# vliu15/3d-brain-tumor-segmentation

Measured on AMD Instinct MI355X. Metric: training volumes/sec (2ch x 128^3), higher is better.
Workload: dtype f32; 1 GPU; BASELINE configs[1]: 2ch x 128^3, batch 1 per GPU, fp32, full fwd+bwd with Dice+KL+L2 VAE loss + Dice metric + TF-form Adam; CLI-default model (base_filters=32, depth=4, groups=8, reduction=8; 42,174,773 params); parallelism=dp1, global_batch=1

## Files before the change

3d-brain-tumor-segmentation_amd/csrc/groupnorm.hip:

```cpp
#include <stdlib.h>
#include "common.h"
#include "bts_internal.h"
#include "finalize_parts.h"

#define GN_BLOCKS_MAX 256

struct GnGeom {
  int N, C, G, cg, mode;
  long V;
  long E;
  long L;
  int B;
  long span;
  int generic;
};

static int gn_geom(GnGeom& g, int N, long V, int C, int G, int mode) {
  if (N <= 0 || V <= 0 || C <= 0 || G <= 0) return BTS_ERR_SHAPE;
  if (C < G || C % G != 0) return BTS_ERR_SHAPE;
  g.N = N; g.C = C; g.G = G; g.cg = C / G; g.mode = mode; g.V = V; g.E = V * C; g.L = g.E / G;
  if (g.E % G != 0) return BTS_ERR_UNSUPPORTED;
  g.generic = (C % 4 != 0 || (C & (C - 1)) != 0 || C > 1024 || g.L % 4 != 0) ? 1 : 0;
  const long unit = (mode == BTS_GN_SLAB) ? g.L : g.E;
  const int units = (mode == BTS_GN_SLAB) ? N * G : N;
// ... 550 lines not shown
                                                           int C, int G, int cg, int lddy, int mode, int relu) {
  const long f0 = blockIdx.x * (long)blockDim.x + threadIdx.x;
  const int cph = (int)((f0 * 4) % C);
  const bool fixed = ((long)gridDim.x * 1024) % C == 0;
  for (long f = f0; f < total4; f += (long)gridDim.x * blockDim.x) {
    const long i = f * 4;
    const long n = i / E;
    const long r = i - n * E;
    const int c = fixed ? cph : (int)(r % C);
    const long pix = i / C;
    const f32x4 v = *reinterpret_cast<const f32x4*>(x + i);
    const f32x4 d = *reinterpret_cast<const f32x4*>(dy + pix * lddy + c);
    const int gsl = (int)(r / L);
    f32x4 o;
#pragma unroll
    for (int e = 0; e < 4; ++e) {
      const int g = (mode == BTS_GN_SLAB) ? gsl : (c + e) / cg;
      const int idx = (mode == BTS_GN_SLAB) ? g * cg + ((c + e) % cg) : (c + e);
      const float rs = rstd[n * G + g];
      const float xh = (v[e] - mean[n * G + g]) * rs;
      float de = d[e];
      const float ga = gamma[idx];
      if (relu && !(xh * ga + beta[idx] > 0.f)) de = 0.f;
      o[e] = (de * ga - c1[n * G + g] - xh * c2[n * G + g]) * rs;
    }
    *reinterpret_cast<f32x4*>(dx + i) = o;
  }
}

bool bts_gn_slab_blocks_(int N, long V, int C, int G, int* B, long* span) {
  GnGeom g;
  if (gn_geom(g, N, V, C, G, BTS_GN_SLAB) != BTS_OK || g.generic) return false;
  *B = g.B;
  *span = g.span;
  return true;
}
__global__ __launch_bounds__(256) void gn_bwd_apply_slab_stream_kernel(const float* __restrict__ x, const float* __restrict__ dy,
                                                                       float* __restrict__ dx, const float* __restrict__ gamma,
                                                                       const float* __restrict__ beta, const float* __restrict__ mean,
                                                                       const float* __restrict__ rstd, const float* __restrict__ c1,
                                                                       const float* __restrict__ c2, long chunks_per_unit, int cpb,
                                                                       int C, int cg, int G, int relu, int lddy) {
  const long chunk0 = (long)blockIdx.x * cpb;
  const long unit = chunk0 / chunks_per_unit;
  const int g = (int)(unit % G);
  const float m = mean[unit], rs = rstd[unit], k1 = c1[unit], k2 = c2[unit];
  const int c = (threadIdx.x * 4) % C;
  float ga[4], be[4];
#pragma unroll
  for (int e = 0; e < 4; ++e) {
    const int idx = g * cg + ((c + e) % cg);
    ga[e] = gamma[idx];
    be[e] = beta[idx];
  }
  const long off = chunk0 * 1024 + threadIdx.x * 4;
  const long vpc = 1024 / C;
  const long doff = (chunk0 * vpc + (threadIdx.x * 4) / C) * lddy + c;
  const long dstep = vpc * lddy;
  auto one = [&](const f32x4 v, const f32x4 d) {
    f32x4 o;
#pragma unroll
    for (int e = 0; e < 4; ++e) {
      const float xh = (v[e] - m) * rs;
      float de = d[e];
      if (relu && !(xh * ga[e] + be[e] > 0.f)) de = 0.f;
      o[e] = (de * ga[e] - k1 - xh * k2) * rs;
    }
    return o;
  };
  int k = 0;
  for (; k + 1 < cpb; k += 2) {
    const f32x4 v0 = *reinterpret_cast<const f32x4*>(x + off + (long)k * 1024);
    const f32x4 d0 = *reinterpret_cast<const f32x4*>(dy + doff + (long)k * dstep);
    const f32x4 v1 = *reinterpret_cast<const f32x4*>(x + off + (long)(k + 1) * 1024);
    const f32x4 d1 = *reinterpret_cast<const f32x4*>(dy + doff + (long)(k + 1) * dstep);
    *reinterpret_cast<f32x4*>(dx + off + (long)k * 1024) = one(v0, d0);
    *reinterpret_cast<f32x4*>(dx + off + (long)(k + 1) * 1024) = one(v1, d1);
  }
  for (; k < cpb; ++k) {
    const f32x4 v0 = *reinterpret_cast<const f32x4*>(x + off + (long)k * 1024);
    const f32x4 d0 = *reinterpret_cast<const f32x4*>(dy + doff + (long)k * dstep);
    *reinterpret_cast<f32x4*>(dx + off + (long)k * 1024) = one(v0, d0);
  }
}

extern "C" int bts_gn_bwd(const float* x, const float* dy, float* dx, const float* gamma, const float* beta,
                          const float* mean, const float* rstd, float* dgamma, float* dbeta, void* workspace,
                          long workspace_bytes, int N, long V, int C, int lddy, int G, int mode, int relu,
                          int accumulate_params, hipStream_t stream) {
  GnGeom g;
  int r = gn_geom(g, N, V, C, G, mode);
  if (r != BTS_OK) return r;
  if (lddy < C) return BTS_ERR_ALIGN;
  if (workspace == nullptr) return BTS_ERR_WORKSPACE;
  if (g.generic || lddy % 4 != 0) {
    if (workspace_bytes < (long)N * G * 2 * 4 + 64) return BTS_ERR_WORKSPACE;
    float* gc1 = reinterpret_cast<float*>(workspace);
    float* gc2 = gc1 + (long)N * G;
    (void)hipGetLastError(); hipLaunchKernelGGL(gn_bwd_group_generic_kernel, dim3(N * G), dim3(256), 0, stream, x, dy, gamma, beta, mean, rstd, gc1, gc2,
                       g.E, g.L, C, G, g.cg, lddy, mode, relu);
    BTS_LAUNCH_CHECK();
    (void)hipGetLastError(); hipLaunchKernelGGL(gn_bwd_param_generic_kernel, dim3(C), dim3(256), 0, stream, x, dy, gamma, beta, mean, rstd, dgamma, dbeta,
                       N, g.E, g.L, C, G, g.cg, lddy, mode, relu, accumulate_params);
    BTS_LAUNCH_CHECK();
    const long total = (long)N * g.E;
    int gb = (int)((total + 255) / 256);
    if (gb > 8192) gb = 8192;
    (void)hipGetLastError(); hipLaunchKernelGGL(gn_bwd_apply_generic_kernel, dim3(gb), dim3(256), 0, stream, x, dy, dx, gamma, beta, mean, rstd, gc1, gc2,
                       total, g.E, g.L, C, G, g.cg, lddy, mode, relu);
    BTS_LAUNCH_CHECK();
    return BTS_OK;
  }
  if ((((uintptr_t)x) & 15) || (((uintptr_t)dy) & 15) || (((uintptr_t)dx) & 15)) return BTS_ERR_ALIGN;
  const long part_bytes = bts_gn_workspace(N, V, C, G, mode);
  const long extra = (long)N * C * 2 * 8 + (long)N * G * 2 * 4 + 64;
  if (workspace_bytes < part_bytes + extra) return BTS_ERR_WORKSPACE;
  double* partial = reinterpret_cast<double*>(workspace);
  double* scratch = reinterpret_cast<double*>(reinterpret_cast<char*>(workspace) + ((part_bytes + 15) & ~15L));
  float* c1 = reinterpret_cast<float*>(scratch + (long)N * C * 2);
  float* c2 = c1 + (long)N * G;
  const bool slab = (mode == BTS_GN_SLAB);
  (void)hipGetLastError(); hipLaunchKernelGGL(gn_bwd_reduce_kernel, dim3(g.B, slab ? N * G : N), dim3(256), 0, stream, x, dy, gamma, beta, mean,
                     rstd, partial, g.E, g.L, g.span, C, G, g.cg, lddy, mode, relu);
  BTS_LAUNCH_CHECK();
  if (slab && g.cg <= 256 && 256 % g.cg == 0) {
    (void)hipGetLastError(); hipLaunchKernelGGL(gn_bwd_finalize_slab_kernel, dim3(G), dim3(256), 0, stream, partial, gamma, dgamma, dbeta, c1, c2, N, G, g.B,
                       g.cg, (double)g.L, accumulate_params);
    BTS_LAUNCH_CHECK();
  } else {
    (void)hipGetLastError(); hipLaunchKernelGGL(gn_bwd_finalize_a_kernel, dim3((N * C + 3) / 4), dim3(256), 0, stream, partial, scratch, N, g.B, C, G, mode);
    BTS_LAUNCH_CHECK();
    (void)hipGetLastError(); hipLaunchKernelGGL(gn_bwd_finalize_kernel, dim3(1), dim3(256), 0, stream, gamma, dgamma, dbeta, c1, c2, scratch, N, C, G,
                       (double)g.L, accumulate_params);
    BTS_LAUNCH_CHECK();
  }
  if (slab && g.L % 1024 == 0 && 1024 % C == 0) {
    const long cpu = g.L / 1024;
    const int cpb = gn_stream_cpb(cpu);
    const long nblk = (long)N * G * cpu / cpb;
    if (nblk <= 0x7fffffffL) {
      (void)hipGetLastError(); hipLaunchKernelGGL(gn_bwd_apply_slab_stream_kernel, dim3((unsigned)nblk), dim3(256), 0, stream, x, dy, dx, gamma, beta,
                         mean, rstd, c1, c2, cpu, cpb, C, g.cg, G, relu, lddy);
      BTS_LAUNCH_CHECK();
      return BTS_OK;
    }
  }
  const long total4 = (long)N * g.E / 4;
  int blocks = (int)((total4 + 255) / 256);
  if (blocks > 8192) blocks = 8192;
  (void)hipGetLastError(); hipLaunchKernelGGL(gn_bwd_apply_kernel, dim3(blocks), dim3(256), 0, stream, x, dy, dx, gamma, beta, mean, rstd, c1, c2,
                     total4, g.E, g.L, C, G, g.cg, lddy, mode, relu);
  BTS_LAUNCH_CHECK();
  return BTS_OK;
}

extern "C" long bts_gn_bwd_workspace(int N, long V, int C, int G, int mode) {
  const long p = bts_gn_workspace(N, V, C, G, mode);
  if (p < 0) return -1;
  return ((p + 15) & ~15L) + (long)N * C * 2 * 8 + (long)N * G * 2 * 4 + 64;
}
```

3d-brain-tumor-segmentation_amd/layers/resnet.py:

```python
import os

import torch

from .. import ops
from ._base import Layer, Tensor, as_tensor, check_data_format, current_tape, gn_mode_of
from .group_norm import GroupNormalization


class ResnetBlock(Layer):
    def __init__(self, filters, data_format='channels_last', groups=8, reduction=2, l2_scale=1e-5, name=None):
        super(ResnetBlock, self).__init__(name=name)
        self.data_format = check_data_format(data_format)
        self.config = {'filters': filters, 'data_format': data_format, 'reduction': reduction, 'l2_scale': l2_scale,
                       'groups': groups}
        if filters % reduction != 0:
            raise ValueError('Reduction ratio, {}, must be a factor of number of channels, {}.'.format(reduction, filters))
        self.filters = filters
        self.groups = groups
        self.reduction = reduction
        self.l2_scale = l2_scale
        self.norm1 = self.track(GroupNormalization(groups=groups, axis=-1, beta_initializer='zeros',
                                                   gamma_initializer='ones', beta_regularizer=l2_scale,
                                                   gamma_regularizer=l2_scale, name=self.name + '/gn1',
                                                   semantics=gn_mode_of(data_format)))
# ... 70 lines not shown
            return res_, gap_, hbuf_, ch_

        if gate is not None:
            gate.wait_stream(main)
            with torch.cuda.stream(gate):
                res, gap, hbuf, ch = gate_branch(None)
            x.t.record_stream(gate)
            for t in (res, gap, hbuf, ch):
                t.record_stream(main)
        if fused is None:
            if slab:
                c1, m1, r1 = ops.conv_fwd_gn(K3, x.t, wp_c1, self.conv1_b.t, f, g, self.norm1.epsilon)
            else:
                c1 = ops.conv_fwd(K3, x.t, wp_c1, self.conv1_b.t, f)
        if gate is None:
            res, gap, hbuf, ch = gate_branch(res)
        if m1 is None:
            m1, r1 = ops.gn_stats(c1, g, self.norm1._mode, self.norm1.epsilon)
        a = ops.gn_apply(c1, self.norm1.gamma.t, self.norm1.beta.t, m1, r1, g, self.norm1._mode, True)
        if slab:
            c2, m2, r2 = ops.conv_fwd_gn(K3, a, wp_c2, self.conv2_b.t, f, g, self.norm2.epsilon)
        else:
            c2 = ops.conv_fwd(K3, a, wp_c2, self.conv2_b.t, f)
            m2, r2 = ops.gn_stats(c2, g, self.norm2._mode, self.norm2.epsilon)
        if gate is not None:
            main.wait_stream(gate)
        if out is None:
            out = Tensor(torch.empty((n, d, h, w, f), dtype=torch.float32, device=x.t.device))
        wsp = self.spatial_k.t.reshape(-1)
        sp = ops.block_epilogue_fwd(res, c2, out.t, wsp, ch, self.norm2.gamma.t, self.norm2.beta.t, m2, r2, g, self.norm2._mode)
        out.cf = self.data_format == 'channels_first'
        tape = current_tape()
        if tape is not None:
            def backward():
                self._backward(x, out, res, gap, hbuf, ch, sp, c1, m1, r1, a, c2, m2, r2, dup_start, dup_shift)
            tape.record(backward)
        return out

    def _backward(self, x, out, res, gap, hbuf, ch, sp, c1, m1, r1, a, c2, m2, r2, dup_start, dup_shift):
        dout = out.grad
        if dout is None:
            return
        f, g = self.filters, self.groups
        cin = x.shape[-1]
        K1, K3 = ops.K1, ops.K3S1
        n1, n2 = self.norm1, self.norm2
        from .group_norm import group_norm_backward
        gw1, a1 = self.se_w1.grad_slot()
        gw2, a2 = self.se_w2.grad_slot()
        gws, a3 = self.spatial_k.grad_slot()
        main = torch.cuda.current_stream()
        gate = ops.side_stream('gate')
        fused = None
        if n2._mode == ops.GN_SLAB and n2.gamma is not None and n2.beta is not None and os.environ.get('BTS_FUSE_BLOCK_BWD', '1') != '0':
            fused = self._fused_gate_gn2_backward(dout, res, c2, sp, gap, hbuf, ch, m2, r2, (gw1, a1), (gw2, a2), (gws, a3))

        def gate_backward():
            acc_ = a1
            if not (a1 == a2 == a3):
                for buf, ac in ((gw1, a1), (gw2, a2), (gws, a3)):
                    if not ac:
                        ops.fill(buf, 0.0)
                acc_ = True
            return ops.se_bwd(dout, res, sp, gap, hbuf, ch, self.se_w1.t, self.se_w2.t, self.spatial_k.t.reshape(-1), gw1, gw2,
                              gws.reshape(-1), accumulate_params=acc_)

        if fused is not None:
            dres, dc2 = fused
            gate = None
        elif gate is not None:
            gate.wait_stream(main)
            with torch.cuda.stream(gate):
                dres = gate_backward()
            for t in (dout, res, sp, gap, hbuf, ch):
                t.record_stream(gate)
            dres.record_stream(main)
        if fused is None:
            dc2 = group_norm_backward(n2, c2, dout, n2.gamma.t, n2.beta.t, m2, r2, True)
        wpb2 = self.packed('c2_b', K3, ops.ROLE_BWD, self.conv2_k, f, f)
        da = torch.empty_like(a)
        ops.conv_bwd_data(K3, dc2, wpb2, da, False)
        _wgrad(K3, a, dc2, self.conv2_k, self.conv2_b)
        del dc2
        dc1 = group_norm_backward(n1, c1, da, n1.gamma.t, n1.beta.t, m1, r1, True)
        del da
        need_dx = x.requires_grad
        if fused is not None:
            pass
        elif gate is None:
            dres = gate_backward()
        else:
            main.wait_stream(gate)
        if need_dx:
            dx, acc = x.grad_slot()
            wpb1 = self.packed('c1_b', K3, ops.ROLE_BWD, self.conv1_k, self.cin_ref, f, cin, dup_start, dup_shift)
            wpbp = self.packed('pt_b', K1, ops.ROLE_BWD, self.ptwise_k, self.cin_ref, f, cin, dup_start, dup_shift)
            ops.conv_bwd_data_pair(dc1, wpb1, dres, wpbp, dx, acc)
        _wgrad(K3, x.t, dc1, self.conv1_k, self.conv1_b, dup_start, dup_shift)
        del dc1
        _wgrad(K1, x.t, dres, self.ptwise_k, self.ptwise_b, dup_start, dup_shift)

    def _fused_gate_gn2_backward(self, dout, res, c2, sp, gap, hbuf, ch, m2, r2, s1, s2, s3):
        n2 = self.norm2
        (gw1, a1), (gw2, a2), (gws, a3) = s1, s2, s3
        if not (torch.is_tensor(dout) and dout.shape[-1] == self.filters):
            return None
        if not ops.block_bwd_takes(res, self.se_w1.t.shape[1], n2.groups, dout, c2):
            return None
        dg, ag = n2.gamma.grad_slot()
        db, ab = n2.beta.grad_slot()
        if not (a1 == a2 == a3):
            for buf, ac in ((gw1, a1), (gw2, a2), (gws, a3)):
                if not ac:
                    ops.fill(buf, 0.0)
            a1 = True
        if ag != ab:
            if not ag:
                ops.fill(dg, 0.0)
            if not ab:
                ops.fill(db, 0.0)
            ag = True
        out = ops.block_bwd(dout, res, c2, sp, gap, hbuf, ch, self.se_w1.t, self.se_w2.t, self.spatial_k.t.reshape(-1), n2.gamma.t, n2.beta.t,
                            m2, r2, n2.groups, gw1, gw2, gws.reshape(-1), dg, db, accumulate_gate_params=a1, accumulate_norm_params=ag)
        if out is None:
            raise RuntimeError('ops.block_bwd declined a block ops.block_bwd_takes accepted')
        return out

    def get_config(self):
        return self.config


def _wgrad(kind, x, dy, kparam, bparam, dup_start=0, dup_shift=0):
    side = ops.side_stream()
    if side is None:
        return _wgrad_here(kind, x, dy, kparam, bparam, dup_start, dup_shift)
    side.wait_stream(torch.cuda.current_stream())
    with torch.cuda.stream(side):
        _wgrad_here(kind, x, dy, kparam, bparam, dup_start, dup_shift)
    for t in (x, dy):
        t.record_stream(side)


def _wgrad_here(kind, x, dy, kparam, bparam, dup_start=0, dup_shift=0):
    dw, aw = kparam.grad_slot()
    db, ab = (None, aw) if bparam is None else bparam.grad_slot()
    if bparam is not None and aw != ab:
        if not aw:
            ops.fill(dw, 0.0)
        if not ab:
            ops.fill(db, 0.0)
        aw = True
    if kind == ops.K3S2T:
        ops.conv_bwd_weight(kind, x, dy, dw, None, accumulate=aw)
        if bparam is not None:
            ops.colsum(dy, sum_over_n=True, out=db, accumulate=aw)
    else:
        ops.conv_bwd_weight(kind, x, dy, dw, db, dup_start, dup_shift, accumulate=aw)
```

3d-brain-tumor-segmentation_amd/ops.py:

```python
import ctypes
import weakref

import numpy as np
import torch

from ._lib import ERRORS, lib

K1, K3S1, K3S2, K3S2T = 0, 1, 2, 3
ROLE_FWD, ROLE_BWD = 0, 1
FLAG_SIGMOID, FLAG_ACCUM = 1, 2
GN_SLAB, GN_CHANNEL = 0, 1

_workspaces = {}

_CFG = {0: '2,1,4,1', 1: '2,2,4,1', 2: '1,2,2,2', 3: '1,1,2,2', 4: '1,1,4,1'}


_VARIANTS = {33: {1: '<0,5>', 2: '<0,4>', 3: '<1,5>', 4: '<1,4>'},
             32: {1: '<3x3x3>', 2: '<1x1x1>'}}


def kernel_symbol(sym, detail=False):
    var, sym = sym >> 16, sym & 0xffff
    if var and detail and sym in _VARIANTS:
        return kernel_symbol(sym) + _VARIANTS[sym].get(var, '<%d>' % var)
    if sym == 20:
        return 'upm_kernel'
    if sym == 21:
        return 'k1s_kernel'
    if sym == 22:
        return 'dsc_kernel'
    if sym == 23:
        return 'wino_kernel'
    if sym == 24:
        return 'wgw_kernel'
    if sym == 25:
        return 'c2_kernel'
    if sym == 26:
        return 'k1w_kernel'
    if sym == 27:
        return 'w3_kernel'
    if sym == 30:
        return 'lp_conv_s1_kernel'
    if sym == 31:
        return 'lp_conv_gather_kernel'
    if sym == 32:
        return 'lp_wgrad_kernel'
    if sym == 33:
        return 'lp_s1d_kernel'
    if sym == 34:
        return 'lp_k1_kernel'
    if sym == 35:
        return 'lp_up_kernel'
    if sym == 36:
        return 'lp_wgs_kernel'
    if sym == 37:
        return 'lp_wgd_kernel'
    if sym == 38:
        return 'lp_s1z_kernel'
    if sym == 39:
        return 'lp_s2t_kernel'
    if sym == 40:
        return 'lp_c2_kernel'
    if sym >= 100:
        return 'wgrad_kernel<%d,%d>' % ((sym - 100) >> 2, (sym - 100) & 3)
    return 'igemm_kernel<%s,%d>' % (_CFG[sym & 7], 4 if sym & 8 else 1)


def profile_enable(on):
    lib().call('bts_profile_enable', 1 if on else 0)


def profile_records(detail=False):
    L = lib()
    out = []
    sym, fl, ms = ctypes.c_int(), ctypes.c_double(), ctypes.c_float()
    for i in range(L._bts_profile_count()):
        L.call('bts_profile_get', i, ctypes.byref(sym), ctypes.byref(fl), ctypes.byref(ms))
        out.append((kernel_symbol(sym.value, detail), fl.value, ms.value))
    return out


def conv_bwd_data_pair(dy, wp_bwd, dy2, wp2_bwd, dx, accumulate):
    n, d, h, w, cin = dx.shape
    cout = dy.shape[4]
    nb = lib().query('bts_conv3d_bwd_data_pair_workspace', n, d, h, w, cin, cout)
    ws = workspace(nb, dy.device) if nb > 0 else None
    lib().call('bts_conv3d_bwd_data_pair', _p(dy), _p(wp_bwd), _p(dy2), _p(wp2_bwd), _p(dx), _p(ws), nb, n, d, h, w, cin,
               ld_of(dx), cout, ld_of(dy), ld_of(dy2), FLAG_ACCUM if accumulate else 0, _stream())
    return dx


def conv_flops(kind, n, d, h, w, cin, cout):
    v = n * d * h * w
    if kind == K1:
        return 2.0 * cin * cout * v
    if kind == K3S2:
        return 2.0 * 27 * cin * cout * (v // 8)
    return 2.0 * 27 * cin * cout * v


def _p(t):
    return None if t is None else ctypes.c_void_p(t.data_ptr())


def _stream():
    return ctypes.c_void_p(torch.cuda.current_stream().cuda_stream)


_side = {}
_side_enabled = True


_fence = {}


def step_fence(kind='train', depth=2):
    import os
    if not torch.cuda.is_available() or os.environ.get('BTS_STEP_FENCE') == '0':
        return
    key = (torch.cuda.current_device(), kind)
    q = _fence.setdefault(key, [])
    while len(q) >= depth:
        q.pop(0).synchronize()
# ... 176 lines not shown
    return c1, res


def conv_fwd_gn(kind, x, wp, bias, cout, groups, eps):
    n, d, h, w, cin = x.shape
    y = torch.empty(conv_out_shape(kind, x.shape, cout), dtype=torch.float32, device=x.device)
    mean = torch.empty(n * groups, dtype=torch.float32, device=x.device)
    rstd = torch.empty(n * groups, dtype=torch.float32, device=x.device)
    nb = lib().query('bts_conv3d_fwd_gn_workspace', kind, n, d, h, w, cin, cout, groups)
    ws = workspace(nb, x.device)
    lib().call('bts_conv3d_fwd_gn', kind, _p(x), _p(wp), _p(bias), _p(y), _p(ws), nb, n, d, h, w, cin, ld_of(x), cout, groups,
               float(eps), _p(mean), _p(rstd), _stream())
    return y, mean, rstd


def conv_fwd_fused2_gn(x, wp3, bias3, wp1, bias1, cout, groups, eps):
    n, d, h, w, cin = x.shape
    if not lib()._bts_conv3d_fwd_can_fuse(n, d, h, w, cin, cout):
        return None
    c1 = torch.empty((n, d, h, w, cout), dtype=torch.float32, device=x.device)
    res = torch.empty_like(c1)
    mean = torch.empty(n * groups, dtype=torch.float32, device=x.device)
    rstd = torch.empty(n * groups, dtype=torch.float32, device=x.device)
    nb = lib().query('bts_conv3d_fwd_gn_workspace', K3S1, n, d, h, w, cin, cout, groups)
    ws = workspace(nb, x.device)
    lib().call('bts_conv3d_fwd_fused2_gn', _p(x), _p(wp3), _p(bias3), _p(c1), _p(wp1), _p(bias1), _p(res), _p(ws), nb, n, d, h, w,
               cin, ld_of(x), cout, cout, groups, float(eps), _p(mean), _p(rstd), _stream())
    return c1, res, mean, rstd


def conv_bwd_data(kind, dy, wp_bwd, dx, accumulate):
    n, d, h, w, cin = dx.shape
    cout = dy.shape[4]
    nb = lib().query('bts_conv3d_bwd_data_workspace', kind, n, d, h, w, cin, cout)
    ws = workspace(nb, dy.device) if nb > 0 else None
    if True:
        lib().call('bts_conv3d_bwd_data', kind, _p(dy), _p(wp_bwd), _p(dx), _p(ws), nb, n, d, h, w, cin, ld_of(dx), cout,
                   ld_of(dy), FLAG_ACCUM if accumulate else 0, _stream())
    return dx


def conv_bwd_weight(kind, x, dy, dw, db, dup_start=0, dup_shift=0, accumulate=False):
    n, d, h, w, cin = x.shape
    cout = dy.shape[4]
    nb = lib().query('bts_conv3d_bwd_weight_workspace', kind, n, d, h, w, cin, cout)
    ws = workspace(nb, x.device)
    if True:
        lib().call('bts_conv3d_bwd_weight', kind, _p(x), _p(dy), _p(dw), _p(db), _p(ws), nb, n, d, h, w, cin, ld_of(x),
                   cout, ld_of(dy), dup_start, dup_shift, 1 if accumulate else 0, _stream())


def gn_stats(x, groups, mode, eps=1e-5):
    if not x.is_contiguous():
        raise RuntimeError('GroupNormalization statistics need a dense tensor')
    n, c = x.shape[0], x.shape[4]
    v = x.shape[1] * x.shape[2] * x.shape[3]
    nb = lib().query('bts_gn_workspace', n, v, c, groups, mode)
    ws = workspace(nb, x.device)
    mean = torch.empty(n * groups, dtype=torch.float32, device=x.device)
    rstd = torch.empty_like(mean)
    lib().call('bts_gn_stats', _p(x), _p(mean), _p(rstd), _p(ws), nb, n, v, c, groups, mode, eps, _stream())
    return mean, rstd


def gn_apply(x, gamma, beta, mean, rstd, groups, mode, relu, out=None):
    n, c = x.shape[0], x.shape[4]
    v = x.shape[1] * x.shape[2] * x.shape[3]
    if out is None:
        out = torch.empty_like(x)
    lib().call('bts_gn_apply', _p(x), _p(out), _p(gamma), _p(beta), _p(mean), _p(rstd), n, v, c, ld_of(out), groups, mode,
               1 if relu else 0, _stream())
    return out


def gn_bwd(x, dy, gamma, beta, mean, rstd, dgamma, dbeta, groups, mode, relu, accumulate_params=False):
    n, c = x.shape[0], x.shape[4]
    v = x.shape[1] * x.shape[2] * x.shape[3]
    nb = lib().query('bts_gn_bwd_workspace', n, v, c, groups, mode)
    ws = workspace(nb, x.device)
    dx = torch.empty_like(x)
    lib().call('bts_gn_bwd', _p(x), _p(dy), _p(dx), _p(gamma), _p(beta), _p(mean), _p(rstd), _p(dgamma), _p(dbeta), _p(ws),
               nb, n, v, c, ld_of(dy), groups, mode, 1 if relu else 0, 1 if accumulate_params else 0, _stream())
    return dx


def colsum(x, scale=1.0, sum_over_n=False, out=None, accumulate=False):
    n, c = x.shape[0], x.shape[-1]
    rows = x.numel() // (n * c)
    ld = ld_of(x) if x.dim() == 5 else x.stride(-2)
    nb = lib().query('bts_colsum_workspace', n, rows, c)
    ws = workspace(nb, x.device)
    if out is None:
        out = torch.empty((c,) if sum_over_n else (n, c), dtype=torch.float32, device=x.device)
    lib().call('bts_colsum', _p(x), _p(out), _p(ws), nb, n, rows, c, ld, float(scale), 1 if sum_over_n else 0,
               1 if accumulate else 0, _stream())
    return out


def se_mlp_fwd(gap, w1, w2):
    n, f = gap.shape
    r = w1.shape[1]
    h = torch.empty((n, r), dtype=torch.float32, device=gap.device)
    ch = torch.empty((n, f), dtype=torch.float32, device=gap.device)
    lib().call('bts_se_mlp_fwd', _p(gap), _p(w1), _p(w2), _p(h), _p(ch), n, f, r, _stream())
    return h, ch


def block_epilogue_fwd(res, c2, out, wsp, ch, gamma, beta, mean, rstd, groups, mode):
    n, f = res.shape[0], res.shape[4]
    v = res.shape[1] * res.shape[2] * res.shape[3]
    sp = torch.empty(n * v, dtype=torch.float32, device=res.device)
    lib().call('bts_block_epilogue_fwd', _p(res), _p(c2), _p(out), _p(sp), _p(wsp), _p(ch), _p(gamma), _p(beta), _p(mean),
               _p(rstd), n, v, f, ld_of(out), groups, mode, _stream())
    return sp


def se_bwd(dout, res, sp, gap, h, ch, w1, w2, wsp, dw1, dw2, dwsp, accumulate_params=False):
    n, f = res.shape[0], res.shape[4]
    v = res.shape[1] * res.shape[2] * res.shape[3]
    r = w1.shape[1]
    nb = lib().query('bts_se_bwd_workspace', n, v, f, r)
    ws = workspace(nb, res.device)
    dres = torch.empty_like(res)
    ds = torch.empty(n * v, dtype=torch.float32, device=res.device)
    dgap = torch.empty((n, f), dtype=torch.float32, device=res.device)
    lib().call('bts_se_bwd', _p(dout), _p(res), _p(sp), _p(gap), _p(h), _p(ch), _p(w1), _p(w2), _p(wsp), _p(dres), _p(ds),
               _p(dgap), _p(dw1), _p(dw2), _p(dwsp), _p(ws), nb, n, v, f, r, ld_of(dout), 1 if accumulate_params else 0,
               _stream())
    return dres


def block_bwd_takes(res, r, groups, dout, c2):
    n, f = res.shape[0], res.shape[4]
    v = res.shape[1] * res.shape[2] * res.shape[3]
    return (lib().probe('bts_block_bwd_workspace', n, v, f, r, groups) >= 0 and ld_of(dout) % 4 == 0 and res.is_contiguous()
            and c2.is_contiguous() and all(t.data_ptr() % 16 == 0 for t in (dout, res, c2)))


def block_bwd(dout, res, c2, sp, gap, h, ch, w1, w2, wsp, gamma, beta, mean, rstd, groups, dw1, dw2, dwsp, dgamma, dbeta,
              accumulate_gate_params=False, accumulate_norm_params=False):
    n, f = res.shape[0], res.shape[4]
    v = res.shape[1] * res.shape[2] * res.shape[3]
    r = w1.shape[1]
    nb = lib().probe('bts_block_bwd_workspace', n, v, f, r, groups)
    if not block_bwd_takes(res, r, groups, dout, c2):
        return None
    ws = workspace(nb, res.device)
    dres = torch.empty_like(res)
    dc2 = torch.empty_like(c2)
    ds = torch.empty(n * v, dtype=torch.float32, device=res.device)
    dgap = torch.empty((n, f), dtype=torch.float32, device=res.device)
    lib().call('bts_block_bwd', _p(dout), ld_of(dout), _p(res), _p(c2), _p(sp), _p(gap), _p(h), _p(ch), _p(w1), _p(w2), _p(wsp), _p(gamma), _p(beta),
               _p(mean), _p(rstd), _p(dres), _p(dc2), _p(ds), _p(dgap), _p(dw1), _p(dw2), _p(dwsp), _p(dgamma), _p(dbeta), _p(ws), nb, n, v, f, r,
               groups, 1 if accumulate_gate_params else 0, 1 if accumulate_norm_params else 0, _stream())
    return dres, dc2


def dropout_mask(shape, rate, seed, device):
    m = torch.empty(shape, dtype=torch.uint8, device=device)
    lib().call('bts_dropout_mask', _p(m), m.numel(), float(rate), int(seed) & (2 ** 64 - 1), _stream())
    return m


def dropout_apply(x, mask, rate):
    y = torch.empty_like(x)
    lib().call('bts_dropout_apply', _p(x), _p(mask), _p(y), x.numel(), float(rate), _stream())
# ... 851 lines not shown
```

include/bts_hip.h:

```cpp
#ifndef BTS_HIP_H
#define BTS_HIP_H
#include <stdint.h>
#ifdef __cplusplus
extern "C" {
#endif

typedef struct ihipStream_t* bts_stream_t;

#define BTS_OK 0
#define BTS_ERR_SHAPE (-1)
#define BTS_ERR_ALIGN (-2)
#define BTS_ERR_UNSUPPORTED (-3)
#define BTS_ERR_WORKSPACE (-4)
#define BTS_ERR_RCCL_BASE (-100)

#define BTS_CONV_K1 0
#define BTS_CONV_K3S1 1
#define BTS_CONV_K3S2 2
#define BTS_CONV_K3S2T 3
#define BTS_ROLE_FWD 0
#define BTS_ROLE_BWD_DATA 1
#define BTS_CONV_FLAG_SIGMOID 1
#define BTS_CONV_FLAG_ACCUM 2

#define BTS_GN_SLAB 0
#define BTS_GN_CHANNEL 1


long bts_conv_packed_floats(int kind, int role, int Cin, int Cout);
int bts_conv_pack(int kind, int role, const float* w, float* wp, int Cin_ref, int Cout, int Cin_slab, int dup_start,
                  int dup_shift, bts_stream_t stream);
long bts_conv_pack_desc_bytes(void);
long bts_conv_pack_desc(void* host_table, int index, long first_block, int kind, int role, const float* w, float* wp,
                        int Cin_ref, int Cout, int Cin_slab, int dup_start, int dup_shift);
int bts_conv_pack_batch(const void* table_dev, const void* table_host, int n, long total_blocks, bts_stream_t stream);
long bts_conv_pack_generation(void);
int bts_conv_pack_forget(const float* wp);
long bts_conv3d_fwd_workspace(int kind, int N, int D, int H, int W, int Cin, int Cout);
int bts_conv3d_fwd(int kind, const float* x, const float* wp_fwd, const float* bias, float* y, void* workspace,
                   long workspace_bytes, int N, int D, int H, int W, int Cin, int ldx, int Cout, int ldy, int flags,
                   bts_stream_t stream);
int bts_conv3d_fwd_can_fuse(int N, int D, int H, int W, int Cin, int Cout);
int bts_conv3d_fwd_fused2(const float* x, const float* wp_fwd, const float* bias, float* y, const float* wp2,
                          const float* bias2, float* y2, int N, int D, int H, int W, int Cin, int ldx, int Cout, int ldy,
                          int ldy2, bts_stream_t stream);
long bts_conv3d_bwd_data_workspace(int kind, int N, int D, int H, int W, int Cin, int Cout);
int bts_conv3d_bwd_data(int kind, const float* dy, const float* wp_bwd, float* dx, void* workspace, long workspace_bytes,
                        int N, int D, int H, int W, int Cin, int lddx, int Cout, int lddy, int flags, bts_stream_t stream);
int bts_conv3d_fwd_config(int kind, int N, int D, int H, int W, int Cin, int Cout);
int bts_conv3d_bwd_data_config(int kind, int N, int D, int H, int W, int Cin, int Cout);
int bts_conv3d_kernel(int dir, int kind, int N, int D, int H, int W, int Cin, int ldx, int Cout, int ldy, int flags, int second,
                      int ld2, int G, int aligned, long workspace_bytes);
long bts_conv3d_bwd_weight_workspace(int kind, int N, int D, int H, int W, int Cin, int Cout);
int bts_conv3d_bwd_weight(int kind, const float* x, const float* dy, float* dw, float* db, void* workspace,
                          long workspace_bytes, int N, int D, int H, int W, int Cin, int ldx, int Cout, int lddy,
                          int dup_start, int dup_shift, int accumulate, bts_stream_t stream);

long bts_gn_workspace(int N, long V, int C, int G, int mode);
long bts_gn_bwd_workspace(int N, long V, int C, int G, int mode);
int bts_gn_stats(const float* x, float* mean, float* rstd, void* workspace, long workspace_bytes, int N, long V, int C,
                 int G, int mode, float eps, bts_stream_t stream);
int bts_gn_apply(const float* x, float* y, const float* gamma, const float* beta, const float* mean, const float* rstd,
                 int N, long V, int C, int ldy, int G, int mode, int relu, bts_stream_t stream);
int bts_gn_bwd(const float* x, const float* dy, float* dx, const float* gamma, const float* beta, const float* mean,
               const float* rstd, float* dgamma, float* dbeta, void* workspace, long workspace_bytes, int N, long V, int C,
               int lddy, int G, int mode, int relu, int accumulate_params, bts_stream_t stream);

long bts_colsum_workspace(int N, long rows, int C);
int bts_colsum(const float* x, float* out, void* workspace, long workspace_bytes, int N, long rows, int C, int ld,
               float scale, int sum_over_n, int accumulate, bts_stream_t stream);
int bts_se_mlp_fwd(const float* gap, const float* w1, const float* w2, float* h, float* ch, int N, int F, int R,
                   bts_stream_t stream);
int bts_block_epilogue_fwd(const float* res, const float* c2, float* out, float* sp, const float* wsp, const float* ch,
                           const float* gamma, const float* beta, const float* mean, const float* rstd, int N, long V,
                           int F, int ldo, int G, int mode, bts_stream_t stream);
long bts_se_bwd_workspace(int N, long V, int F, int R);
int bts_se_bwd(const float* dout, const float* res, const float* sp, const float* gap, const float* h, const float* ch,
               const float* w1, const float* w2, const float* wsp, float* dres, float* ds, float* dgap, float* dw1,
               float* dw2, float* dwsp, void* workspace, long workspace_bytes, int N, long V, int F, int R, int lddo,
               int accumulate_params, bts_stream_t stream);

long bts_block_bwd_workspace(int N, long V, int F, int R, int G);
int bts_block_bwd(const float* dout, int lddo, const float* res, const float* c2, const float* sp, const float* gap, const float* h,
                  const float* ch, const float* w1, const float* w2, const float* wsp, const float* gamma, const float* beta,
                  const float* mean, const float* rstd, float* dres, float* dc2, float* ds, float* dgap, float* dw1, float* dw2,
                  float* dwsp, float* dgamma, float* dbeta, void* workspace, long workspace_bytes, int N, long V, int F, int R, int G,
                  int accumulate_gate_params, int accumulate_norm_params, bts_stream_t stream);

int bts_dropout_mask(uint8_t* mask, long n, float rate, uint64_t seed, bts_stream_t stream);
int bts_dropout_apply(const float* x, const uint8_t* mask, float* y, long n, float rate, bts_stream_t stream);
int bts_normal(float* out, long n, uint64_t seed, bts_stream_t stream);
int bts_vae_sample_fwd(const float* proj, const float* eps, float* z, int N, int L, bts_stream_t stream);
int bts_vae_sample_bwd(const float* proj, const float* eps, const float* dz, float* dproj, int N, int L, bts_stream_t stream);
int bts_fill(float* p, long n, float v, bts_stream_t stream);
int bts_axpy(float* y, const float* x, long n, float a, bts_stream_t stream);
int bts_add_strided(float* dst, const float* src, long rows, int C, int ldd, int lds_, int accumulate, bts_stream_t stream);
int bts_scalar_lincomb(float* out, const float* a, const float* b, float ca, float cb, bts_stream_t stream);
int bts_relu_bwd(const float* y, const float* dy, float* dx, long n, bts_stream_t stream);
int bts_sigmoid_bwd(const float* y, const float* dy, float* dx, long rows, int C, int ldy, int lddy, bts_stream_t stream);

long bts_dense_workspace(int N, int in, int out);
int bts_dense_fwd(const float* x, const float* w, const float* bias, float* y, void* workspace, long workspace_bytes, int N,
                  int in, int out, int relu, bts_stream_t stream);
int bts_dense_bwd(const float* x, const float* w, const float* g, float* dx, float* dw, float* db, int N, int in, int out,
                  int accumulate_dx, int accumulate_params, bts_stream_t stream);

long bts_loss_workspace(void);
int bts_loss_sums(const float* y_pred, const float* y, const float* x, const float* y_vae, const float* proj, double* sums,
                  void* workspace, long workspace_bytes, int N, long V, int C, int ldp, int ldy, int Cx, int ldx, int ldv,
                  int Lz, bts_stream_t stream);
int bts_loss_value(const double* sums, float* loss, float* parts, int C, int has_vae, bts_stream_t stream);
int bts_loss_bwd(const float* y_pred, const float* y, const float* x, const float* y_vae, const float* proj,
                 const double* sums, const float* gscale, float* dlogit, float* dyvae, float* dproj, int N, long V, int C,
                 int ldp, int ldy, int Cx, int ldx, int ldv, int Lz, int through_sigmoid, bts_stream_t stream);
int bts_dice_metric_sums(const float* y_true, const float* y_pred, uint8_t* labels, double* table, int N, long V, int W,
                         int C, int ldt, int ldp, int channels_last_axes, bts_stream_t stream);
int bts_dice_metric_value(const double* table, float* out, int W, int C, int channels_last_axes, bts_stream_t stream);
long bts_l2_workspace(void);
int bts_l2_reg_fwd(const float* params, const long* off, const long* len, const float* coef, int nranges, float* out,
                   void* workspace, long workspace_bytes, bts_stream_t stream);
int bts_l2_reg_bwd(const float* params, float* grads, const long* off, const long* len, const float* coef, int nranges,
                   const float* gscale, bts_stream_t stream);

int bts_adam_tf_step(float* p, const float* g, float* m, float* v, long n, float lr_t, float beta1, float beta2, float eps,
                     float gmul, bts_stream_t stream);
int bts_grad_nonfinite(const float* g, long n, int* flag, bts_stream_t stream);
int bts_adam_tf_step_guarded(float* p, const float* g, float* m, float* v, long n, float lr_t, float beta1, float beta2, float eps,
                             float gmul, const int* skip, bts_stream_t stream);

long bts_conv3d_bwd_data_pair_workspace(int N, int D, int H, int W, int Cin, int Cout);
int bts_conv3d_bwd_data_pair(const float* dy, const float* wp_bwd, const float* dy2, const float* wp2_bwd, float* dx,
                             void* workspace, long workspace_bytes, int N, int D, int H, int W, int Cin, int lddx, int Cout,
                             int lddy, int lddy2, int flags, bts_stream_t stream);

long bts_conv3d_fwd_gn_workspace(int kind, int N, int D, int H, int W, int Cin, int Cout, int G);
int bts_conv3d_fwd_gn(int kind, const float* x, const float* wp_fwd, const float* bias, float* y, void* workspace,
                      long workspace_bytes, int N, int D, int H, int W, int Cin, int ldx, int Cout, int G, float eps, float* mean,
                      float* rstd, bts_stream_t stream);
int bts_conv3d_fwd_fused2_gn(const float* x, const float* wp_fwd, const float* bias, float* y, const float* wp2,
                             const float* bias2, float* y2, void* workspace, long workspace_bytes, int N, int D, int H, int W,
                             int Cin, int ldx, int Cout, int ldy2, int G, float eps, float* mean, float* rstd,
                             bts_stream_t stream);

int bts_maxpool2_fwd(const float* x, float* y, uint8_t* idx, int N, int D, int H, int W, int C, int ldx, int ldy,
                     bts_stream_t stream);
int bts_maxpool2_bwd(const float* dy, const uint8_t* idx, float* dx, int N, int D, int H, int W, int C, int lddy, int lddx,
                     int accumulate, bts_stream_t stream);
int bts_upsample2_fwd(const float* x, float* y, int N, int D, int H, int W, int C, int ldx, int ldy, bts_stream_t stream);
int bts_upsample2_bwd(const float* dy, float* dx, int N, int D, int H, int W, int C, int lddy, int lddx, int accumulate,
// ... 208 lines not shown
```

Baseline: 27.32 volumes/s.

## Fuse GroupNorm backward apply into thin-input conv3d weight-gradient kernel

```diff
diff --git a/3d-brain-tumor-segmentation_amd/csrc/groupnorm.hip b/3d-brain-tumor-segmentation_amd/csrc/groupnorm.hip
--- a/3d-brain-tumor-segmentation_amd/csrc/groupnorm.hip
+++ b/3d-brain-tumor-segmentation_amd/csrc/groupnorm.hip
@@ -656,6 +656,34 @@
     const f32x4 d0 = *reinterpret_cast<const f32x4*>(dy + doff + (long)k * dstep);
     *reinterpret_cast<f32x4*>(dx + off + (long)k * 1024) = one(v0, d0);
   }
+}
+
+static int gn_bwd_sums(const GnGeom& g, const float* x, const float* dy, const float* gamma, const float* beta, const float* mean,
+                       const float* rstd, float* dgamma, float* dbeta, void* workspace, long part_bytes, int lddy, int relu,
+                       int accumulate_params, float** c1_out, float** c2_out, hipStream_t stream) {
+  const int N = g.N, C = g.C, G = g.G, mode = g.mode;
+  double* partial = reinterpret_cast<double*>(workspace);
+  double* scratch = reinterpret_cast<double*>(reinterpret_cast<char*>(workspace) + ((part_bytes + 15) & ~15L));
+  float* c1 = reinterpret_cast<float*>(scratch + (long)N * C * 2);
+  float* c2 = c1 + (long)N * G;
+  const bool slab = (mode == BTS_GN_SLAB);
+  (void)hipGetLastError(); hipLaunchKernelGGL(gn_bwd_reduce_kernel, dim3(g.B, slab ? N * G : N), dim3(256), 0, stream, x, dy, gamma, beta, mean,
+                     rstd, partial, g.E, g.L, g.span, C, G, g.cg, lddy, mode, relu);
+  BTS_LAUNCH_CHECK();
+  if (slab && g.cg <= 256 && 256 % g.cg == 0) {
+    (void)hipGetLastError(); hipLaunchKernelGGL(gn_bwd_finalize_slab_kernel, dim3(G), dim3(256), 0, stream, partial, gamma, dgamma, dbeta, c1, c2, N, G, g.B,
+                       g.cg, (double)g.L, accumulate_params);
+    BTS_LAUNCH_CHECK();
+  } else {
+    (void)hipGetLastError(); hipLaunchKernelGGL(gn_bwd_finalize_a_kernel, dim3((N * C + 3) / 4), dim3(256), 0, stream, partial, scratch, N, g.B, C, G, mode);
+    BTS_LAUNCH_CHECK();
+    (void)hipGetLastError(); hipLaunchKernelGGL(gn_bwd_finalize_kernel, dim3(1), dim3(256), 0, stream, gamma, dgamma, dbeta, c1, c2, scratch, N, C, G,
+                       (double)g.L, accumulate_params);
+    BTS_LAUNCH_CHECK();
+  }
+  *c1_out = c1;
+  *c2_out = c2;
+  return BTS_OK;
 }
 
 extern "C" int bts_gn_bwd(const float* x, const float* dy, float* dx, const float* gamma, const float* beta,
@@ -689,25 +717,10 @@
   const long part_bytes = bts_gn_workspace(N, V, C, G, mode);
   const long extra = (long)N * C * 2 * 8 + (long)N * G * 2 * 4 + 64;
   if (workspace_bytes < part_bytes + extra) return BTS_ERR_WORKSPACE;
-  double* partial = reinterpret_cast<double*>(workspace);
-  double* scratch = reinterpret_cast<double*>(reinterpret_cast<char*>(workspace) + ((part_bytes + 15) & ~15L));
-  float* c1 = reinterpret_cast<float*>(scratch + (long)N * C * 2);
-  float* c2 = c1 + (long)N * G;
+  float *c1, *c2;
+  r = gn_bwd_sums(g, x, dy, gamma, beta, mean, rstd, dgamma, dbeta, workspace, part_bytes, lddy, relu, accumulate_params, &c1, &c2, stream);
+  if (r != BTS_OK) return r;
   const bool slab = (mode == BTS_GN_SLAB);
-  (void)hipGetLastError(); hipLaunchKernelGGL(gn_bwd_reduce_kernel, dim3(g.B, slab ? N * G : N), dim3(256), 0, stream, x, dy, gamma, beta, mean,
-                     rstd, partial, g.E, g.L, g.span, C, G, g.cg, lddy, mode, relu);
-  BTS_LAUNCH_CHECK();
-  if (slab && g.cg <= 256 && 256 % g.cg == 0) {
-    (void)hipGetLastError(); hipLaunchKernelGGL(gn_bwd_finalize_slab_kernel, dim3(G), dim3(256), 0, stream, partial, gamma, dgamma, dbeta, c1, c2, N, G, g.B,
-                       g.cg, (double)g.L, accumulate_params);
-    BTS_LAUNCH_CHECK();
-  } else {
-    (void)hipGetLastError(); hipLaunchKernelGGL(gn_bwd_finalize_a_kernel, dim3((N * C + 3) / 4), dim3(256), 0, stream, partial, scratch, N, g.B, C, G, mode);
-    BTS_LAUNCH_CHECK();
-    (void)hipGetLastError(); hipLaunchKernelGGL(gn_bwd_finalize_kernel, dim3(1), dim3(256), 0, stream, gamma, dgamma, dbeta, c1, c2, scratch, N, C, G,
-                       (double)g.L, accumulate_params);
-    BTS_LAUNCH_CHECK();
-  }
   if (slab && g.L % 1024 == 0 && 1024 % C == 0) {
     const long cpu = g.L / 1024;
     const int cpb = gn_stream_cpb(cpu);
@@ -733,3 +746,283 @@
   if (p < 0) return -1;
   return ((p + 15) & ~15L) + (long)N * C * 2 * 8 + (long)N * G * 2 * 4 + 64;
 }
+
+#define GWT_TX 32
+#define GWT_TY 4
+#define GWT_TZ 4
+#define GWT_HX (GWT_TX + 2)
+#define GWT_HY (GWT_TY + 2)
+#define GWT_HZ (GWT_TZ + 2)
+#define GWT_HALO (GWT_HZ * GWT_HY * GWT_HX)
+#define GWT_MAX_WGS 2048
+
+struct GwtParams {
+  const float* c1;
+  const float* da;
+  const float* x;
+  const float *gamma, *beta, *mean, *rstd, *k1, *k2;
+  float* partial;
+  int N, D, H, W, Cin, ldx, C, ldda, G, cg, relu;
+  int L;
+  int ntx, nty, ntz, ntiles, tiles_per_wg;
+  int buf_floats;
+  int st_off;
+};
+
+template <int MT>
+__global__ __launch_bounds__(256, MT <= 2 ? 4 : 2) void gn_bwd_apply_wgrad_thin_kernel(const GwtParams p) {
+  extern __shared__ __attribute__((aligned(16))) float gwt_lds[];
+  __shared__ float gam_s[32], bet_s[32];
+  const int tid = threadIdx.x, lane = tid & 63, wave = tid >> 6;
+  const int kk = lane >> 5, nn = lane & 31;
+  const int Cin = p.Cin, C = p.C;
+  const int one_off = p.st_off - 4;
+  if (tid < 32) {
+    gam_s[tid] = tid < C ? p.gamma[tid] : 0.f;
+    bet_s[tid] = tid < C ? p.beta[tid] : 0.f;
+  }
+  int aoff[MT], amul[MT];
+#pragma unroll
+  for (int mt = 0; mt < MT; ++mt) {
+    const int m = mt * 32 + nn;
+    if (m < 27 * Cin) {
+      const int t = m / Cin, ci = m - t * Cin;
+      const int kz = t / 9, ky = (t / 3) % 3, kx = t % 3;
+      aoff[mt] = ((kz * GWT_HY + ky) * GWT_HX + kx) * Cin + ci;
+      amul[mt] = 1;
+    } else {
+      aoff[mt] = (m == 27 * Cin) ? one_off : one_off + 1;
+      amul[mt] = 0;
+    }
+  }
+  f32x16 acc[MT];
+#pragma unroll
+  for (int mt = 0; mt < MT; ++mt)
+#pragma unroll
+    for (int r = 0; r < 16; ++r) acc[mt][r] = 0.f;
+  const long V = (long)p.D * p.H * p.W;
+  const int cgm = nn & (p.cg - 1);
+  const int tile0 = blockIdx.x * p.tiles_per_wg;
+  for (int it = 0; it < p.tiles_per_wg; ++it) {
+    const int tile = tile0 + it;
+    if (tile >= p.ntiles) break;
+    int r = tile;
+    const int tx = r % p.ntx; r /= p.ntx;
+    const int ty = r % p.nty; r /= p.nty;
+    const int tz = r % p.ntz;
+    const int n = r / p.ntz;
+    const int x0 = tx * GWT_TX, y0 = ty * GWT_TY, z0 = tz * GWT_TZ;
+    float* buf = gwt_lds + (it & 1) * p.buf_floats;
+    const float* xn = p.x + (long)n * V * p.ldx;
+    for (int i = tid; i < GWT_HALO * Cin; i += 256) {
+      const int vox = i / Cin, ci = i - vox * Cin;
+      const int hx = vox % GWT_HX, hy = (vox / GWT_HX) % GWT_HY, hz = vox / (GWT_HX * GWT_HY);
+      const int gx = x0 - 1 + hx, gy = y0 - 1 + hy, gz = z0 - 1 + hz;
+      float v = 0.f;
+      if (gx >= 0 && gx < p.W && gy >= 0 && gy < p.H && gz >= 0 && gz < p.D)
+        v = xn[(((long)gz * p.H + gy) * p.W + gx) * p.ldx + ci];
+      buf[i] = v;
+    }
+    if (tid < 4) buf[one_off + tid] = tid == 0 ? 1.f : 0.f;
+    if (tid < p.G * 4) {
+      const int g = tid >> 2, w = tid & 3;
+      const float* src = w == 0 ? p.mean : w == 1 ? p.rstd : w == 2 ? p.k1 : p.k2;
+      buf[p.st_off + tid] = src[n * p.G + g];
+    }
+    __syncthreads();
+    const int z = z0 + wave;
+    if (z < p.D) {
+      const int ny = (p.H - y0 < GWT_TY) ? p.H - y0 : GWT_TY;
+      const int nch = ny * 4;
+      const long vplane = ((long)z * p.H + y0) * p.W + x0;
+      const float* cpl = p.c1 + ((long)n * V + vplane) * C;
+      const float* dpl = p.da + ((long)n * V + vplane) * p.ldda;
+      const bool cok = nn < C;
+      const bool relu = p.relu != 0;
+      auto load = [&](int ch, float (&cv)[4], float (&dv)[4]) {
+        const int yy = ch >> 2, q = ch & 3;
+        const unsigned vo = (unsigned)(yy * p.W + q * 8 + kk);
+#pragma unroll
+        for (int s = 0; s < 4; ++s) {
+          const bool ok = cok && (x0 + q * 8 + 2 * s + kk < p.W);
+          cv[s] = ok ? cpl[(vo + 2 * s) * (unsigned)C + nn] : 0.f;
+          dv[s] = ok ? dpl[(vo + 2 * s) * (unsigned)p.ldda + nn] : 0.f;
+        }
+      };
+      float cn[4], dn[4];
+      load(0, cn, dn);
+      int flat = 0, g = 0, lim = 0;
+#pragma unroll 1
+      for (int ch = 0; ch < nch; ++ch) {
+        float cv[4], dv[4];
+#pragma unroll
+        for (int s = 0; s < 4; ++s) { cv[s] = cn[s]; dv[s] = dn[s]; }
+        if (ch + 1 < nch) load(ch + 1, cn, dn);
+        const int yy = ch >> 2, q = ch & 3;
+        if (q == 0) {
+          flat = (int)(vplane + (long)yy * p.W + kk) * C + nn;
+          g = flat / p.L;
+          lim = (g + 1) * p.L;
+        }
+        const int vb0 = ((wave * GWT_HY + yy) * GWT_HX + q * 8 + kk) * Cin;
+#pragma unroll
+        for (int s = 0; s < 4; ++s) {
+          const bool ok = cok && (x0 + q * 8 + 2 * s + kk < p.W);
+          const int gs = ok ? g : 0;
+          const f32x4 st = *reinterpret_cast<const f32x4*>(buf + p.st_off + gs * 4);
+          const int gi = ok ? gs * p.cg + cgm : 0;
+          const float ga = gam_s[gi], be = bet_s[gi];
+          const float m = st[0], rs = st[1], k1 = st[2], k2 = st[3];
+          const float xh = (cv[s] - m) * rs;
+          const float yv = xh * ga + be;
+          const bool live = (yv > 0.f) | !relu;
+          const float de = live ? dv[s] : 0.f;
+          float o = (de * ga - k1 - xh * k2) * rs;
+          if (!ok) o = 0.f;
+          const int vb = vb0 + 2 * s * Cin;
+#pragma unroll
+          for (int mt = 0; mt < MT; ++mt) {
+            const float a = buf[vb * amul[mt] + aoff[mt]];
+            acc[mt] = __builtin_amdgcn_mfma_f32_32x32x2f32(a, o, acc[mt], 0, 0, 0);
+          }
+          flat += 2 * C;
+          const bool up = flat >= lim;
+          g += up ? 1 : 0;
+          lim += up ? p.L : 0;
+        }
+      }
+    }
+  }
+  for (int w = 1; w < 4; ++w) {
+    __syncthreads();
+    if (wave == w) {
+#pragma unroll
+      for (int mt = 0; mt < MT; ++mt)
+#pragma unroll
+        for (int r = 0; r < 16; ++r) gwt_lds[(mt * 16 + r) * 64 + lane] = acc[mt][r];
+    }
+    __syncthreads();
+    if (wave == 0) {
+#pragma unroll
+      for (int mt = 0; mt < MT; ++mt)
+#pragma unroll
+        for (int r = 0; r < 16; ++r) acc[mt][r] += gwt_lds[(mt * 16 + r) * 64 + lane];
+    }
+  }
+  if (wave == 0) {
+    float* dst = p.partial + (long)blockIdx.x * (MT * 1024);
+#pragma unroll
+    for (int mt = 0; mt < MT; ++mt)
+#pragma unroll
+      for (int r = 0; r < 16; ++r) {
+        const int row = mt * 32 + (r & 3) + 8 * (r >> 2) + 4 * kk;
+        dst[row * 32 + nn] = acc[mt][r];
+      }
+  }
+}
+
+__global__ __launch_bounds__(1024) void gn_bwd_apply_wgrad_thin_finalize_kernel(const float* __restrict__ partial, float* dw, float* db, int nwg,
+                                                                                int wg_stride, int rows, int C, int accum) {
+  __shared__ double sh[32][33];
+  const int m = blockIdx.x, co = threadIdx.x & 31, sl = threadIdx.x >> 5;
+  const float* src = partial + m * 32 + co;
+  double a0 = 0.0, a1 = 0.0, a2 = 0.0, a3 = 0.0;
+  int w = sl;
+  for (; w + 96 < nwg; w += 128) {
+    const float v0 = src[(long)w * wg_stride], v1 = src[(long)(w + 32) * wg_stride];
+    const float v2 = src[(long)(w + 64) * wg_stride], v3 = src[(long)(w + 96) * wg_stride];
+    a0 += (double)v0; a1 += (double)v1; a2 += (double)v2; a3 += (double)v3;
+  }
+  for (; w < nwg; w += 32) a0 += (double)src[(long)w * wg_stride];
+  sh[sl][co] = (a0 + a1) + (a2 + a3);
+  __syncthreads();
+  if (sl == 0 && co < C) {
+    double t = sh[0][co];
+#pragma unroll
+    for (int k = 1; k < 32; ++k) t += sh[k][co];
+    float* d = (m < rows - 1) ? dw + (long)m * C + co : (db ? db + co : nullptr);
+    if (d) *d = accum ? (*d + (float)t) : (float)t;
+  }
+}
+
+struct GwtPlan {
+  GnGeom g;
+  int MT, nwg, tiles_per_wg, ntx, nty, ntz, ntiles, buf_floats, st_off;
+  long gn_bytes, part_bytes, partial_off, total;
+  size_t shmem;
+};
+
+static int gwt_plan(GwtPlan& pl, int N, int D, int H, int W, int Cin, int C, int G) {
+  if (N <= 0 || D <= 0 || H <= 0 || W <= 0 || Cin <= 0 || C <= 0 || G <= 0) return BTS_ERR_SHAPE;
+  const long V = (long)D * H * W;
+  int r = gn_geom(pl.g, N, V, C, G, BTS_GN_SLAB);
+  if (r != BTS_OK) return r;
+  if (pl.g.generic || Cin > 4 || C > 32 || G > 32 || V * C >= (1L << 30) || (long)N * V >= (1L << 31) || pl.g.L < 2 * C) return BTS_ERR_UNSUPPORTED;
+  pl.MT = (27 * Cin + 1 + 31) / 32;
+  pl.ntx = (W + GWT_TX - 1) / GWT_TX; pl.nty = (H + GWT_TY - 1) / GWT_TY; pl.ntz = (D + GWT_TZ - 1) / GWT_TZ;
+  const long nt = (long)N * pl.ntz * pl.nty * pl.ntx;
+  if (nt >= (1L << 30)) return BTS_ERR_UNSUPPORTED;
+  pl.ntiles = (int)nt;
+  const int want = pl.ntiles < GWT_MAX_WGS ? pl.ntiles : GWT_MAX_WGS;
+  pl.tiles_per_wg = (pl.ntiles + want - 1) / want;
+  pl.nwg = (pl.ntiles + pl.tiles_per_wg - 1) / pl.tiles_per_wg;
+  pl.st_off = ((GWT_HALO * Cin + 3) & ~3) + 4;
+  pl.buf_floats = pl.st_off + G * 4;
+  pl.shmem = (size_t)2 * pl.buf_floats * sizeof(float);
+  if (pl.shmem < (size_t)pl.MT * 1024 * sizeof(float)) pl.shmem = (size_t)pl.MT * 1024 * sizeof(float);
+  pl.part_bytes = bts_gn_workspace(N, V, C, G, BTS_GN_SLAB);
+  pl.gn_bytes = bts_gn_bwd_workspace(N, V, C, G, BTS_GN_SLAB);
+  if (pl.part_bytes < 0 || pl.gn_bytes < 0) return BTS_ERR_UNSUPPORTED;
+  pl.partial_off = (pl.gn_bytes + 15) & ~15L;
+  pl.total = pl.partial_off + (long)pl.nwg * pl.MT * 1024 * 4;
+  return BTS_OK;
+}
+
+int bts_prof_on();
+void bts_prof_begin(int sym, double flops, hipStream_t stream);
+void bts_prof_end(hipStream_t stream);
+
+extern "C" long bts_gn_bwd_apply_conv3d_bwd_weight_thin_workspace(int N, int D, int H, int W, int Cin, int C, int G) {
+  GwtPlan pl;
+  if (gwt_plan(pl, N, D, H, W, Cin, C, G) != BTS_OK) return -1;
+  return pl.total;
+}
+
+extern "C" int bts_gn_bwd_apply_conv3d_bwd_weight_thin(const float* c1, const float* da, const float* x, const float* gamma, const float* beta,
+                                                       const float* mean, const float* rstd, float* dgamma, float* dbeta, float* dw, float* db,
+                                                       void* workspace, long workspace_bytes, int N, int D, int H, int W, int Cin, int ldx,
+                                                       int C, int ldda, int G, int relu, int accumulate_norm_params,
+                                                       int accumulate_conv_params, hipStream_t stream) {
+  GwtPlan pl;
+  int r = gwt_plan(pl, N, D, H, W, Cin, C, G);
+  if (r != BTS_OK) return r;
+  if (ldx < Cin || ldda < C) return BTS_ERR_ALIGN;
+  if (ldda % 4 != 0) return BTS_ERR_UNSUPPORTED;
+  if ((((uintptr_t)c1) & 15) || (((uintptr_t)da) & 15)) return BTS_ERR_ALIGN;
+  if (workspace == nullptr || workspace_bytes < pl.total) return BTS_ERR_WORKSPACE;
+  if (((uintptr_t)workspace) & 15) return BTS_ERR_ALIGN;
+  float *k1, *k2;
+  r = gn_bwd_sums(pl.g, c1, da, gamma, beta, mean, rstd, dgamma, dbeta, workspace, pl.part_bytes, ldda, relu, accumulate_norm_params, &k1, &k2,
+                  stream);
+  if (r != BTS_OK) return r;
+  GwtParams p;
+  p.c1 = c1; p.da = da; p.x = x; p.gamma = gamma; p.beta = beta; p.mean = mean; p.rstd = rstd; p.k1 = k1; p.k2 = k2;
+  p.partial = reinterpret_cast<float*>(reinterpret_cast<char*>(workspace) + pl.partial_off);
+  p.N = N; p.D = D; p.H = H; p.W = W; p.Cin = Cin; p.ldx = ldx; p.C = C; p.ldda = ldda; p.G = G; p.cg = pl.g.cg; p.relu = relu;
+  p.L = (int)pl.g.L;
+  p.ntx = pl.ntx; p.nty = pl.nty; p.ntz = pl.ntz; p.ntiles = pl.ntiles; p.tiles_per_wg = pl.tiles_per_wg;
+  p.buf_floats = pl.buf_floats; p.st_off = pl.st_off;
+  typedef void (*GwtKernel)(const GwtParams);
+  static const GwtKernel kernels[4] = {gn_bwd_apply_wgrad_thin_kernel<1>, gn_bwd_apply_wgrad_thin_kernel<2>, gn_bwd_apply_wgrad_thin_kernel<3>,
+                                       gn_bwd_apply_wgrad_thin_kernel<4>};
+  const bool prof = bts_prof_on();
+  if (prof) bts_prof_begin(28, 2.0 * (27.0 * Cin + 1.0) * C * (double)N * D * H * W, stream);
+  (void)hipGetLastError(); hipLaunchKernelGGL(kernels[pl.MT - 1], dim3(pl.nwg), dim3(256), pl.shmem, stream, p);
+  if (prof) bts_prof_end(stream);
+  BTS_LAUNCH_CHECK();
+  const int rows = 27 * Cin + 1;
+  (void)hipGetLastError(); hipLaunchKernelGGL(gn_bwd_apply_wgrad_thin_finalize_kernel, dim3(rows), dim3(1024), 0, stream, p.partial, dw, db, pl.nwg,
+                     pl.MT * 1024, rows, C, accumulate_conv_params);
+  BTS_LAUNCH_CHECK();
+  return BTS_OK;
+}
diff --git a/3d-brain-tumor-segmentation_amd/layers/resnet.py b/3d-brain-tumor-segmentation_amd/layers/resnet.py
--- a/3d-brain-tumor-segmentation_amd/layers/resnet.py
+++ b/3d-brain-tumor-segmentation_amd/layers/resnet.py
@@ -176,9 +176,12 @@
         ops.conv_bwd_data(K3, dc2, wpb2, da, False)
         _wgrad(K3, a, dc2, self.conv2_k, self.conv2_b)
         del dc2
-        dc1 = group_norm_backward(n1, c1, da, n1.gamma.t, n1.beta.t, m1, r1, True)
-        del da
         need_dx = x.requires_grad
+        thin_tail = (not need_dx and dup_shift == 0 and n1.gamma is not None and n1.beta is not None and
+                     ops.gn_bwd_wgrad_thin_takes(x.t, c1, da, g, n1._mode))
+        if not thin_tail:
+            dc1 = group_norm_backward(n1, c1, da, n1.gamma.t, n1.beta.t, m1, r1, True)
+            del da
         if fused is not None:
             pass
         elif gate is None:
@@ -190,6 +193,10 @@
             wpb1 = self.packed('c1_b', K3, ops.ROLE_BWD, self.conv1_k, self.cin_ref, f, cin, dup_start, dup_shift)
             wpbp = self.packed('pt_b', K1, ops.ROLE_BWD, self.ptwise_k, self.cin_ref, f, cin, dup_start, dup_shift)
             ops.conv_bwd_data_pair(dc1, wpb1, dres, wpbp, dx, acc)
+        if thin_tail:
+            _wgrad(K1, x.t, dres, self.ptwise_k, self.ptwise_b, dup_start, dup_shift)
+            _gn_bwd_wgrad_thin(n1, x.t, c1, da, m1, r1, self.conv1_k, self.conv1_b)
+            return
         _wgrad(K3, x.t, dc1, self.conv1_k, self.conv1_b, dup_start, dup_shift)
         del dc1
         _wgrad(K1, x.t, dres, self.ptwise_k, self.ptwise_b, dup_start, dup_shift)
@@ -235,6 +242,27 @@
         t.record_stream(side)
 
 
+def _gn_bwd_wgrad_thin(norm, x, c1, da, mean, rstd, kparam, bparam):
+    dg, ag = norm.gamma.grad_slot()
+    dbt, ab = norm.beta.grad_slot()
+    if ag != ab:
+        if not ag:
+            ops.fill(dg, 0.0)
+        if not ab:
+            ops.fill(dbt, 0.0)
+        ag = True
+    dw, aw = kparam.grad_slot()
+    db, acb = bparam.grad_slot()
+    if aw != acb:
+        if not aw:
+            ops.fill(dw, 0.0)
+        if not acb:
+            ops.fill(db, 0.0)
+        aw = True
+    ops.gn_bwd_wgrad_thin(x, c1, da, norm.gamma.t, norm.beta.t, mean, rstd, dg, dbt, dw, db, norm.groups, True,
+                          accumulate_norm_params=ag, accumulate_conv_params=aw)
+
+
 def _wgrad_here(kind, x, dy, kparam, bparam, dup_start=0, dup_shift=0):
     dw, aw = kparam.grad_slot()
     db, ab = (None, aw) if bparam is None else bparam.grad_slot()
diff --git a/3d-brain-tumor-segmentation_amd/ops.py b/3d-brain-tumor-segmentation_amd/ops.py
--- a/3d-brain-tumor-segmentation_amd/ops.py
+++ b/3d-brain-tumor-segmentation_amd/ops.py
@@ -40,6 +40,8 @@
         return 'k1w_kernel'
     if sym == 27:
         return 'w3_kernel'
+    if sym == 28:
+        return 'gn_bwd_apply_wgrad_thin_kernel'
     if sym == 30:
         return 'lp_conv_s1_kernel'
     if sym == 31:
@@ -382,6 +384,28 @@
     lib().call('bts_gn_bwd', _p(x), _p(dy), _p(dx), _p(gamma), _p(beta), _p(mean), _p(rstd), _p(dgamma), _p(dbeta), _p(ws),
                nb, n, v, c, ld_of(dy), groups, mode, 1 if relu else 0, 1 if accumulate_params else 0, _stream())
     return dx
+
+
+def gn_bwd_wgrad_thin_takes(x, c1, da, groups, mode):
+    import os
+    if mode != GN_SLAB or os.environ.get('BTS_GN_WGRAD_THIN', '1') == '0':
+        return False
+    n, d, h, w, cin = x.shape
+    c = c1.shape[4]
+    if cin > 4 or not c1.is_contiguous() or ld_of(da) % 4 != 0 or (c1.data_ptr() | da.data_ptr()) & 15:
+        return False
+    return lib().probe('bts_gn_bwd_apply_conv3d_bwd_weight_thin_workspace', n, d, h, w, cin, c, groups) >= 0
+
+
+def gn_bwd_wgrad_thin(x, c1, da, gamma, beta, mean, rstd, dgamma, dbeta, dw, db, groups, relu, accumulate_norm_params=False,
+                      accumulate_conv_params=False):
+    n, d, h, w, cin = x.shape
+    c = c1.shape[4]
+    nb = lib().query('bts_gn_bwd_apply_conv3d_bwd_weight_thin_workspace', n, d, h, w, cin, c, groups)
+    ws = workspace(nb, x.device)
+    lib().call('bts_gn_bwd_apply_conv3d_bwd_weight_thin', _p(c1), _p(da), _p(x), _p(gamma), _p(beta), _p(mean), _p(rstd), _p(dgamma),
+               _p(dbeta), _p(dw), _p(db), _p(ws), nb, n, d, h, w, cin, ld_of(x), c, ld_of(da), groups, 1 if relu else 0,
+               1 if accumulate_norm_params else 0, 1 if accumulate_conv_params else 0, _stream())
 
 
 def colsum(x, scale=1.0, sum_over_n=False, out=None, accumulate=False):
diff --git a/include/bts_hip.h b/include/bts_hip.h
--- a/include/bts_hip.h
+++ b/include/bts_hip.h
@@ -65,6 +65,12 @@
 int bts_gn_bwd(const float* x, const float* dy, float* dx, const float* gamma, const float* beta, const float* mean,
                const float* rstd, float* dgamma, float* dbeta, void* workspace, long workspace_bytes, int N, long V, int C,
                int lddy, int G, int mode, int relu, int accumulate_params, bts_stream_t stream);
+long bts_gn_bwd_apply_conv3d_bwd_weight_thin_workspace(int N, int D, int H, int W, int Cin, int C, int G);
+int bts_gn_bwd_apply_conv3d_bwd_weight_thin(const float* c1, const float* da, const float* x, const float* gamma, const float* beta,
+                                            const float* mean, const float* rstd, float* dgamma, float* dbeta, float* dw, float* db,
+                                            void* workspace, long workspace_bytes, int N, int D, int H, int W, int Cin, int ldx, int C,
+                                            int ldda, int G, int relu, int accumulate_norm_params, int accumulate_conv_params,
+                                            bts_stream_t stream);
 
 long bts_colsum_workspace(int N, long rows, int C);
 int bts_colsum(const float* x, float* out, void* workspace, long workspace_bytes, int N, long rows, int C, int ld,
```

Measured after the change: 27.36 volumes/s (median of 6 runs). Within noise of the previous version (+0.1%).
